# kerry-he/fsae-mpc

Measured on AMD Instinct MI355X. Metric: QP solves/sec (batched LTV-MPC, N=40 nx=5 nu=2 fp64), higher is better.
Workload: dtype f64

## Files before the change

### fsae-mpc_amd/csrc/qp_probe.h

```cpp
#pragma once
#include "qp_solve_kernel.h"

template <int T, int NB> __global__ __launch_bounds__(64) void syrk_probe_kernel(QpParams P, int reps) {
  const int b = blockIdx.x;
  extern __shared__ double lds[];
  Ctx k;
  ctx_setup<T>(k, P, b, lds);
  const QpSolveLds L = qp_solve_lds(T, NB, P.d.np);
  double* MB = lds + L.vecs;
  k.ring = MB + L.border + L.tiles; k.cof = k.ring + L.ring;
  for (int js = 0; js < k.JT; ++js) {
    const int ix = js * 64 + k.lane;
    rowp(k, R_D)[ix] = 1.0; rowp(k, R_W1)[ix] = 0.5; rowp(k, R_W2)[ix] = 0.25; rowp(k, R_W3)[ix] = 2.0;
  }
  __syncthreads();
  v4d acc[Tri<T>::NT];
  acc_init<T>(k, acc);
  const unsigned long long t0 = __builtin_amdgcn_s_memtime();
  for (int r = 0; r < reps; ++r) {
    Stream<T> st;
    st.open(k);
    pass_syrk<T, NB>(k, st, acc, vecp(k, V_P1), vecp(k, V_P2), vecp(k, V_P3), MB);
    st.close();
    __syncthreads();
// ... 60 lines not shown
  for (int r = 0; r < reps; ++r) {
    acc_init<T>(k, acc);
#pragma unroll
    for (int K = 0; K < T; ++K) {
#pragma unroll
      for (int p = 0; p < 4; ++p) if (k.q + 4 * p == k.c) acc[Tri<T>::idx(K, K)][p] += 20.0;
    }
    for (int i = k.lane; i < 16 * T; i += 64) RV[i] = 1.0 + (i & 15);
    __syncthreads();
    __builtin_amdgcn_sched_barrier(0);
    unsigned long long t0 = __builtin_amdgcn_s_memtime();
    reg_factor<T, 1>(k, acc, YL, 1e-30);
    __builtin_amdgcn_sched_barrier(0);
    unsigned long long t1 = __builtin_amdgcn_s_memtime();
    tt[0] += t1 - t0;
    v4d Yk, none = {0.0, 0.0, 0.0, 0.0};
#pragma unroll
    for (int K = 0; K < T; ++K) {
#pragma unroll
      for (int p = 0; p < 4; ++p) { Yk[p] = (k.q + 4 * p == k.c) ? 1.0 : 0.0; if (k.q + 4 * p == k.c) acc[Tri<T>::idx(K, K)][p] += 30.0; }
      diag_factor<DiagForm<T, 1>::form>(k, acc[Tri<T>::idx(K, K)], Yk, none, 1e-30);
      cs += Yk[0];
    }
    __builtin_amdgcn_sched_barrier(0);
    unsigned long long t2 = __builtin_amdgcn_s_memtime();
    tt[1] += t2 - t1;
#pragma unroll
    for (int K = 0; K < T; ++K) { tile_store(k, YL + K * 272, acc[Tri<T>::idx(K, K)]); __syncthreads(); acc[Tri<T>::idx(K, K)] = tile_load_t(k, YL + K * 272); }
    __builtin_amdgcn_sched_barrier(0);
    unsigned long long t3 = __builtin_amdgcn_s_memtime();
    tt[2] += t3 - t2;
    double y[T][4];
    vec_forward<T, true>(k, acc, YL, RV, y);
    WAVE_SYNC();
    vec_backward<T, true>(k, acc, YL, y, RV);
    WAVE_SYNC();
// ... 10 lines not shown
```

### fsae-mpc_amd/csrc/qp_rules.h

```cpp
#pragma once
#include <math.h>
#if defined(__HIPCC__)
#include <hip/hip_runtime.h>
#define QPR_HD __host__ __device__ __forceinline__
#else
#define QPR_HD inline
#endif
#ifndef QP_REFINE_ATTEMPTS
#define QP_REFINE_ATTEMPTS 3
#endif
template <int C> struct IC { static constexpr int value = C; };
#define QPR_GAMMA_F 0.99
#define QPR_STEP_BACKOFF 0.99999999
#define QPR_AMAX_UNSET 1e300
#define QPR_AMAX_SET 1e299
#define QPR_CORRECTOR_MIN_STEP 0.05
#define QPR_MU_FLOOR 1e-5
#define QPR_PROGRESS 0.9
#define QPR_STALL_SAVED 5
#define QPR_STALL_UNSAVED 25
#define QPR_DIVERGED_X 1e13
#define QPR_DIVERGED_Z 1e15
#define QPR_INFEASIBLE_RP 1e-6
#define QPR_RHO 1e6
// ... 18 lines not shown
  return o;
}
QPR_HD bool qpr_has_lower(bool valid, double l) { return valid && l > -INFINITY; }
QPR_HD bool qpr_has_upper(bool valid, double u) { return valid && u < INFINITY; }
QPR_HD double qpr_side_affine(double t, double z, double rp, double va, double& a_aff, double& s1, double& s2) {
  const double dt = va + rp, dz = -z - (z / t) * dt;
  if (dt < 0) a_aff = fmin(a_aff, -t / dt);  if (dz < 0) a_aff = fmin(a_aff, -z / dz);
  s1 += t * dz + z * dt; s2 += dt * dz;
  return dt * dz / t;
}
struct QprDir { double dt, dz; };
QPR_HD QprDir qpr_side_step(double t, double z, double rp, double va, double dv, double smu, double cw) {
  const double dta = va + rp, dza = -z - (z / t) * dta;
  const double c = smu - cw * dta * dza;
  QprDir o; o.dt = dv + rp; o.dz = -z + c / t - (z / t) * o.dt;
  return o;
}
struct QprBlock { double amax, bp, bdp, bd, bdd; };
QPR_HD QprBlock qpr_block_none() { QprBlock b; b.amax = QPR_AMAX_UNSET; b.bp = 0; b.bdp = 0; b.bd = 0; b.bdd = 0; return b; }
QPR_HD void qpr_side_block(double t, double z, const QprDir& d, QprBlock& b, double& q1, double& q2) {
  if (d.dt < 0 && -t / d.dt < b.amax) { b.amax = -t / d.dt; b.bp = t; b.bdp = d.dt; b.bd = z; b.bdd = d.dz; }
  if (d.dz < 0 && -z / d.dz < b.amax) { b.amax = -z / d.dz; b.bp = z; b.bdp = d.dz; b.bd = t; b.bdd = d.dt; }
  q1 += t * d.dz + z * d.dt; q2 += d.dt * d.dz;
}
struct QprCenter { double mu_aff, sigma, smu, cw; };
QPR_HD QprCenter qpr_centering(double gap, double cnt, double mu, double a_aff, double s1, double s2, double tol, double fval) {
  QprCenter o; o.mu_aff = fmax(0.0, gap + a_aff * (s1 + a_aff * s2)) / cnt;
  double sigma = mu > 0 ? (o.mu_aff / mu) * (o.mu_aff / mu) * (o.mu_aff / mu) : 0.0;
  if (sigma > 1.0) sigma = 1.0;
  const double mu_floor = QPR_MU_FLOOR * tol * fmax(1.0, fabs(fval)) / cnt;
// ... 97 lines not shown
```

### fsae-mpc_amd/csrc/qp_selftest.h

```cpp
#pragma once
#include <stdlib.h>
#include <stdio.h>
#include "qp_solve_kernel.h"

namespace {

__global__ void mfma_selftest_kernel(const double* Am, const double* Bm, double* Cm) {
  const int lane = threadIdx.x;
  const double a = Am[(lane & 15) * 4 + (lane >> 4)];
  const double bb = Bm[(lane >> 4) * 16 + (lane & 15)];
  v4d c = {0, 0, 0, 0};
  c = __builtin_amdgcn_mfma_f64_16x16x4f64(a, bb, c, 0, 0, 0);
#pragma unroll
  for (int p = 0; p < 4; ++p) Cm[((lane >> 4) + 4 * p) * 16 + (lane & 15)] = c[p];
}

DEVINL bool same_bits(double a, double b) { return __double_as_longlong(a) == __double_as_longlong(b) || (a != a && b != b); }
template <class OP> DEVINL double lds_grp16(double* sh, int lane, double v) {
  const int src[4] = {lane ^ 1, lane ^ 2, (lane & ~7) | (7 - (lane & 7)), (lane & ~15) | (15 - (lane & 15))};
#pragma unroll
  for (int s = 0; s < 4; ++s) {
    sh[lane] = v; __syncthreads();
    const double o = sh[src[s]]; __syncthreads();
    v = OP::f(v, o);
// ... 72 lines not shown
      double a[4] = {x[4], x[5], x[6], x[7]};
      wave_sum(a);
      int nb = 0;
#pragma unroll
      for (int i = 0; i < 4; ++i) nb += same_bits(a[i], wave_sum_zf(x[4 + i])) ? 0 : 1;
      if (nb && first < 0) first = 100 * 65;
      bad += nb;
    }
    if (bad != before && first_round < 0) first_round = r;
  }
  if (bad) {
    if (atomicAdd(&out[0], bad) == 0) { out[1] = first; out[2] = first_round; out[3] = lane; }
  }
}

template <int FORM> DEVINL int diag_factor_bad_vs_old(const Ctx& k, const v4d& U0, const v4d& R0, double floor_abs, const v4d& Uo, const v4d& Yo, const v4d& Ro, int bo) {
  v4d U = U0, R = R0, Y;
#pragma unroll
  for (int p = 0; p < 4; ++p) Y[p] = (k.q + 4 * p == k.c) ? 1.0 : 0.0;
  const int b = diag_factor<FORM>(k, U, Y, R, floor_abs);
  int bad = (b != bo) ? 1 : 0;
#pragma unroll
  for (int p = 0; p < 4; ++p)
    bad += (__double_as_longlong(U[p]) != __double_as_longlong(Uo[p])) + (__double_as_longlong(Y[p]) != __double_as_longlong(Yo[p])) +
           (__double_as_longlong(R[p]) != __double_as_longlong(Ro[p]));
  return bad;
}
__global__ __launch_bounds__(64) void diag_factor_selftest_kernel(const double* __restrict__ in, int ntiles, double floor_abs, int* __restrict__ out) {
  Ctx k = {};
  k.lane = threadIdx.x; k.c = k.lane & 15; k.q = k.lane >> 4;
  int bad = 0, first = -1, form = 0;
  for (int t = 0; t < ntiles; ++t) {
    v4d U0, R0, Uo, Ro, Yo;
#pragma unroll
    for (int p = 0; p < 4; ++p) {
      U0[p] = in[(size_t)t * 512 + (k.q + 4 * p) * 16 + k.c];
      R0[p] = in[(size_t)t * 512 + 256 + (k.q + 4 * p) * 16 + k.c];
      Yo[p] = (k.q + 4 * p == k.c) ? 1.0 : 0.0;
    }
    Uo = U0; Ro = R0;
    const int bo = diag_factor<0>(k, Uo, Yo, Ro, floor_abs);
    const int b1 = diag_factor_bad_vs_old<1>(k, U0, R0, floor_abs, Uo, Yo, Ro, bo);
    const int b2 = diag_factor_bad_vs_old<2>(k, U0, R0, floor_abs, Uo, Yo, Ro, bo);
    if ((b1 | b2) && first < 0) { first = t; form = b1 ? 1 : 2; }
    bad += b1 + b2;
  }
  if (bad) {
    if (atomicAdd(&out[0], bad) == 0) { out[1] = first; out[2] = form; out[3] = k.lane; }
  }
}

template <int T, int NB> __global__ __launch_bounds__(64) void initial_point_selftest_kernel(QpParams P, int* __restrict__ out) {
  extern __shared__ double lds[];
  Ctx k;
  (void)ctx_setup<T>(k, P, 0, lds);
  const QpSolveLds L = qp_solve_lds(T, NB, P.d.np);
  k.ring = lds + L.vecs + L.border + L.tiles;
  k.cof = k.ring + L.ring;
// ... 88 lines not shown
  (void)hipMemset(dout, 0, sizeof(hout));
  free(h);
  hipLaunchKernelGGL(lane_reduce_selftest_kernel, dim3(1), dim3(64), 0, 0, d, rounds, dout);
  hipError_t e = hipDeviceSynchronize();
  if (e == hipSuccess) e = hipMemcpy(hout, dout, sizeof(hout), hipMemcpyDeviceToHost);
  (void)hipFree(d); (void)hipFree(dout);
  if (e != hipSuccess) { snprintf(msg, msglen, "lane-reduce selftest: %s", hipGetErrorString(e)); return -1; }
  if (hout[0]) snprintf(msg, msglen, "lane reductions: %d mismatches, first: test %d (1/2/4/8: grp16 single / batched, 16: q, 64: wave, 65: wave_sum batch) op %d (sum/max/min) round %d lane %d",
                        hout[0], hout[1] / 100, hout[1] % 100, hout[2], hout[3]);
  return hout[0];
}

int qp_selftest_diag_factor(char* msg, int msglen) {
  const int ntiles = 64;
  const double floor_abs = 1e-9;
  double* h = (double*)malloc(sizeof(double) * ntiles * 512);
  if (!h) return -1;
  unsigned long long st = 0xD1B54A32D192ED03ull;
  auto rnd = [&]() { st = st * 6364136223846793005ull + 1442695040888963407ull; return ((unsigned)(st >> 33)) / 2147483648.0; };
  for (int t = 0; t < ntiles; ++t) {
    double* D = h + (size_t)t * 512; double* R = D + 256;
    double Q[16][16], sv[16];
    for (int i = 0; i < 16; ++i) for (int j = 0; j < 16; ++j) Q[i][j] = i == j ? 1.0 : 0.0;
    for (int r = 0; r < 3; ++r) {
      double v[16], vv = 0;
      for (int i = 0; i < 16; ++i) { v[i] = 2.0 * rnd() - 1.0; vv += v[i] * v[i]; }
      for (int i = 0; i < 16; ++i) {
        double qv = 0;
        for (int j = 0; j < 16; ++j) qv += Q[i][j] * v[j];
        for (int j = 0; j < 16; ++j) Q[i][j] -= 2.0 * qv * v[j] / vv;
      }
    }
    const double lc = 10.0 * (t < 61 ? t / 60.0 : 0.3);
    for (int i = 0; i < 16; ++i) sv[i] = pow(10.0, -lc * i / 15.0);
    for (int i = 0; i < 16; ++i) for (int j = 0; j < 16; ++j) {
      double a = 0;
      for (int l = 0; l < 16; ++l) a += Q[i][l] * sv[l] * Q[j][l];
      D[i * 16 + j] = a;
    }
    for (int i = 0; i < 16; ++i) for (int j = 0; j < i; ++j) D[i * 16 + j] = D[j * 16 + i];
    for (int i = 0; i < 256; ++i) R[i] = 20.0 * rnd() - 10.0;
    if (t == 61) for (int j = 0; j < 16; ++j) { D[6 * 16 + j] *= 1e-6; D[j * 16 + 6] *= 1e-6; }
    if (t == 62) { D[5 * 16 + 9] = NAN; D[9 * 16 + 5] = NAN; }
    if (t == 63) D[10 * 16 + 10] = INFINITY;
  }
  double* d = 0; int* dout = 0; int hout[4] = {0, 0, 0, 0};
  if (hipMalloc(&d, sizeof(double) * ntiles * 512) != hipSuccess || hipMalloc(&dout, sizeof(hout)) != hipSuccess) { free(h); if (d) (void)hipFree(d); return -1; }
  (void)hipMemcpy(d, h, sizeof(double) * ntiles * 512, hipMemcpyHostToDevice);
  (void)hipMemset(dout, 0, sizeof(hout));
  free(h);
  hipLaunchKernelGGL(diag_factor_selftest_kernel, dim3(1), dim3(64), 0, 0, d, ntiles, floor_abs, dout);
  hipError_t e = hipDeviceSynchronize();
  if (e == hipSuccess) e = hipMemcpy(hout, dout, sizeof(hout), hipMemcpyDeviceToHost);
  (void)hipFree(d); (void)hipFree(dout);
  if (e != hipSuccess) { snprintf(msg, msglen, "diag_factor selftest: %s", hipGetErrorString(e)); return -1; }
  if (hout[0]) snprintf(msg, msglen, "diag_factor forms: %d mismatches with the former form, first: tile %d form %d lane %d", hout[0], hout[1], hout[2], hout[3]);
  return hout[0];
}

template <int T, int NB> static hipError_t initial_point_launch(const QpParams& P, int* dout) {
  hipError_t e = hipFuncSetAttribute(reinterpret_cast<const void*>(&initial_point_selftest_kernel<T, NB>), hipFuncAttributeMaxDynamicSharedMemorySize, (int)P.d.lds_solve);
  if (e != hipSuccess) return e;
  hipLaunchKernelGGL((initial_point_selftest_kernel<T, NB>), dim3(1), dim3(64), P.d.lds_solve, 0, P, dout);
// ... 87 lines not shown
```

### fsae-mpc_amd/csrc/qp_solve_kernel.h

```cpp
#pragma once
#include "qp_solver.h"
#include "qp_lane.h"
#include "qp_rules.h"

#ifndef QP_SOLVE_PAIR
#define QP_SOLVE_PAIR 0
#endif
#ifndef QP_DIAG_FLAT
#define QP_DIAG_FLAT 1
#endif
#ifndef QP_SYRK_INTERLEAVE
#define QP_SYRK_INTERLEAVE 0
#endif
#ifndef QP_STARTUP_ATW
#define QP_STARTUP_ATW 0
#endif
#ifndef QP_SWEEP_BATCH
#define QP_SWEEP_BATCH 6
#endif

namespace {

template <int T> struct Tri {
  static constexpr int NT = T * (T + 1) / 2;
  __host__ __device__ static constexpr int idx(int I, int J) { return I * T - (I * (I - 1)) / 2 + (J - I); }
};

struct Ctx {
  int n, m, T, Kq, J, JB, JT, np, lane, c, q, nc, nb, ntr;
  const int* perm; const int* tcs; const int* aoff; const int* tend;
  const double* Aw; const double* Hw; const double* Ab; const double* Hb;
  double* rows;
  double* ring;
// ... 139 lines not shown
  DEVINL void load(const Ctx& k, const double* const* arr, int js) {
    const int jc = js < k.J ? js : k.J - 1;
#pragma unroll
    for (int a = 0; a < NA; ++a) reg[a] = arr[a][jc * 64 + k.lane];
  }
  DEVINL void commit(const Ctx& k) {
#pragma unroll
    for (int a = 0; a < NA; ++a) k.cof[a * 64 + k.lane] = reg[a];
  }
  DEVINL void read_pair(const Ctx& k, int s, v2d* out) const {
#pragma unroll
    for (int a = 0; a < NA; ++a) out[a] = *reinterpret_cast<const v2d*>(k.cof + a * 64 + k.q * 16 + (s & 15));
  }
};

template <int T, int NB> DEVINL void pass_syrk(const Ctx& k, Stream<T>& st, v4d* acc, double* P1, double* P2, double* P3, double* MB) {
  constexpr int NBB = NB > 0 ? NB : 1;
  constexpr int NA = 4 + NB;
  const int JS = k.J * 64;
  const double* arr[NA];
  arr[0] = rowp(k, R_D); arr[1] = rowp(k, R_W1); arr[2] = rowp(k, R_W2); arr[3] = rowp(k, R_W3);
#pragma unroll
  for (int e = 0; e < NB; ++e) arr[4 + e] = k.Ab + (size_t)e * JS;
  double p1[T], p2[T], p3[T];
  double pb[NBB][T], sbb[NBB][NBB], pwb[3][NBB];
#pragma unroll
  for (int t = 0; t < T; ++t) { p1[t] = 0; p2[t] = 0; p3[t] = 0; }
#pragma unroll
  for (int e = 0; e < NBB; ++e) {
#pragma unroll
    for (int t = 0; t < T; ++t) pb[e][t] = 0;
#pragma unroll
    for (int f = 0; f < NBB; ++f) sbb[e][f] = 0;
    pwb[0][e] = pwb[1][e] = pwb[2][e] = 0;
  }
  CoefStage<NA> cs;
  int tr = 0;
  st.start(k);
// ... 7 lines not shown
      for (int u = 0; u < 2; ++u) {
        v2d b[C], cf[NA];
        st.template next_pair<C>(k, b);
        cs.read_pair(k, 4 * tr + 2 * u, cf);
        asm volatile("" ::: "memory");
#if QP_SYRK_INTERLEAVE
        double a2[2][C];
#pragma unroll
        for (int h = 0; h < 2; ++h)
#pragma unroll
          for (int t = 0; t < C; ++t) a2[h][t] = cf[0][h] * b[t][h];
#endif
#pragma unroll
        for (int h = 0; h < 2; ++h) {
          double a[C], ab[NBB];
          const double dd = cf[0][h], w1 = cf[1][h], w2 = cf[2][h], w3 = cf[3][h];
#pragma unroll
          for (int e = 0; e < NB; ++e) ab[e] = cf[4 + e][h];
#pragma unroll
#if QP_SYRK_INTERLEAVE
          for (int t = 0; t < C; ++t) a[t] = a2[h][t];
#else
          for (int t = 0; t < C; ++t) a[t] = dd * b[t][h];
#endif
#pragma unroll
          for (int I = 0; I < C; ++I)
#pragma unroll
            for (int Jt = I; Jt < C; ++Jt)
              acc[Tri<T>::idx(I, Jt)] = __builtin_amdgcn_mfma_f64_16x16x4f64(a[I], b[Jt][h], acc[Tri<T>::idx(I, Jt)], 0, 0, 0);
#pragma unroll
          for (int t = 0; t < C; ++t) {
            p1[t] = fma(w1, b[t][h], p1[t]); p2[t] = fma(w2, b[t][h], p2[t]); p3[t] = fma(w3, b[t][h], p3[t]);
          }
#pragma unroll
          for (int e = 0; e < NB; ++e) {
            const double dab = dd * ab[e];
#pragma unroll
            for (int t = 0; t < C; ++t) pb[e][t] = fma(dab, b[t][h], pb[e][t]);
#pragma unroll
            for (int f = e; f < NB; ++f) sbb[e][f] = fma(dab, ab[f], sbb[e][f]);
            pwb[0][e] = fma(w1, ab[e], pwb[0][e]); pwb[1][e] = fma(w2, ab[e], pwb[1][e]); pwb[2][e] = fma(w3, ab[e], pwb[2][e]);
          }
#if QP_SYRK_INTERLEAVE
#pragma unroll
          for (int i = 0; i < C * (C + 1) / 2; ++i) {
            __builtin_amdgcn_sched_group_barrier(0x008, 1, 0);
            __builtin_amdgcn_sched_group_barrier(0x002, 2, 0);
          }
#endif
        }
      }
    }
  };
  if constexpr (T >= 1) phase(IC<1>{});
  if constexpr (T >= 2) phase(IC<2>{});
  if constexpr (T >= 3) phase(IC<3>{});
  if constexpr (T >= 4) phase(IC<4>{});
  if constexpr (T >= 5) phase(IC<5>{});
  if constexpr (T >= 6) phase(IC<6>{});
  if constexpr (T >= 7) phase(IC<7>{});
  if constexpr (T >= 8) phase(IC<8>{});
  if (k.ntr > 0) st.finish();
#pragma unroll
  for (int t = 0; t < T; ++t) {
    double v1 = q_sum(p1[t]), v2 = q_sum(p2[t]), v3 = q_sum(p3[t]);
    if (k.q == 0) { P1[16 * t + k.c] = v1; P2[16 * t + k.c] = v2; P3[16 * t + k.c] = v3; }
  }
#pragma unroll
  for (int e = 0; e < NB; ++e) {
#pragma unroll
    for (int t = 0; t < T; ++t) { const double vb = q_sum(pb[e][t]); if (k.q == 0) MB[e * k.np + 16 * t + k.c] = vb; }
    const double v1 = q_sum(pwb[0][e]), v2 = q_sum(pwb[1][e]), v3 = q_sum(pwb[2][e]);
    if (k.lane == 0) { P1[k.nc + e] = v1; P2[k.nc + e] = v2; P3[k.nc + e] = v3; }
#pragma unroll
    for (int f = 0; f < NB; ++f) {
      const double sv = q_sum(f >= e ? sbb[e][f] : sbb[f][e]);
      if (k.lane == 0) MB[e * k.np + k.nc + f] = sv;
    }
  }
}

template <int T, int NB, int NVEC, int FUSE> DEVINL void pass_Av(const Ctx& k, Stream<T>& st, const double* const* vin, double* const* rout, double* Pcor, double* Pcor2 = nullptr, const double* const* cfarr = nullptr) {
  constexpr int NBB = NB > 0 ? NB : 1;
  constexpr int NC = FUSE == 1 ? 6 : (FUSE >= 2 ? 3 : (FUSE == -1 ? 1 : 0));
  constexpr int NA = NC + NB;
  const int JS = k.J * 64;
  const double* arr[NA > 0 ? NA : 1];
  if (FUSE == 1) { arr[0] = rowp(k, R_RPL); arr[1] = rowp(k, R_CB1); arr[2] = rowp(k, R_CC1); arr[3] = rowp(k, R_RPU); arr[4] = rowp(k, R_CB2); arr[5] = rowp(k, R_CC2); }
// ... 165 lines not shown
  v4d Z;
#pragma unroll
  for (int p = 0; p < 4; ++p) Z[p] = slot[(k.q + 4 * p) * 17 + k.c];
  return Z;
}
DEVINL v4d tile_load_t(const Ctx& k, const double* slot) {
  v4d Z;
#pragma unroll
  for (int p = 0; p < 4; ++p) Z[p] = slot[k.c * 17 + k.q + 4 * p];
  return Z;
}

DEVINL double on_lanes(unsigned long long mask, double v, double otherwise) {
  return __builtin_amdgcn_inverse_ballot_w64(mask) ? v : otherwise;
}
template <int FORM> DEVINL int diag_factor(const Ctx& k, v4d& Ud, v4d& Yk, v4d& rk, double floor_abs) {
  constexpr bool FLAT = FORM >= 1;
  int bad = 0;
#pragma unroll
  for (int p = 0; p < 4; ++p) {
    const double d00 = rl(Ud[p], 4 * p + 0), d01 = rl(Ud[p], 4 * p + 1), d02 = rl(Ud[p], 4 * p + 2), d03 = rl(Ud[p], 4 * p + 3);
    const double d11 = rl(Ud[p], 16 + 4 * p + 1), d12 = rl(Ud[p], 16 + 4 * p + 2), d13 = rl(Ud[p], 16 + 4 * p + 3);
    const double d22 = rl(Ud[p], 32 + 4 * p + 2), d23 = rl(Ud[p], 32 + 4 * p + 3);
    const double d33 = rl(Ud[p], 48 + 4 * p + 3);
    auto piv = [&](double t) {
      if constexpr (FORM >= 2) {
        const bool low = !(t > floor_abs);
        bad |= (low & !(fabs(t) < INFINITY)) ? 1 : 0;
        t = low ? floor_abs : t;
      } else {
        if (!(t > floor_abs)) { if (!(fabs(t) < INFINITY)) bad = 1; t = floor_abs; }
// ... 14 lines not shown
    if constexpr (FLAT) {
      const unsigned long long L0 = 1ull << (4 * p), L1 = 1ull << (16 + 4 * p), L2 = 1ull << (32 + 4 * p), L3 = 1ull << (48 + 4 * p);
      double wa = on_lanes(L0, i0, 0.0);
      wa = on_lanes(L0 << 1, w10, wa); wa = on_lanes(L0 << 2, w20, wa); wa = on_lanes(L0 << 3, w30, wa);
      wa = on_lanes(L1 << 1, i1, wa); wa = on_lanes(L1 << 2, w21, wa); wa = on_lanes(L1 << 3, w31, wa);
      wa = on_lanes(L2 << 2, i2, wa); wa = on_lanes(L2 << 3, w32, wa);
      wa = on_lanes(L3 << 3, i3, wa);
      const v4d nu = __builtin_amdgcn_mfma_f64_16x16x4f64(wa, Ud[p], z, 0, 0, 0);
      Ud[p] = nu[p];
      double a = 0.0;
      if (p < 3) {
        a = on_lanes(0x0001000100010001ull * (0xFFFFull & (0xFFFFull << (4 * p + 4))), -Ud[p], 0.0);
        Ud = __builtin_amdgcn_mfma_f64_16x16x4f64(a, Ud[p], Ud, 0, 0, 0);
      }
      const v4d ny = __builtin_amdgcn_mfma_f64_16x16x4f64(wa, Yk[p], z, 0, 0, 0);
      const v4d nr = __builtin_amdgcn_mfma_f64_16x16x4f64(wa, rk[p], z, 0, 0, 0);
      Yk[p] = ny[p]; rk[p] = nr[p];
      if (p < 3) {
        Yk = __builtin_amdgcn_mfma_f64_16x16x4f64(a, Yk[p], Yk, 0, 0, 0);
        rk = __builtin_amdgcn_mfma_f64_16x16x4f64(a, rk[p], rk, 0, 0, 0);
      }
      if constexpr (FORM >= 2) asm("" : "+v"(bad));
    } else {
      const int a_ = k.c - 4 * p;
      double wa = 0.0;
      if (k.q == 0) wa = a_ == 0 ? i0 : (a_ == 1 ? w10 : (a_ == 2 ? w20 : (a_ == 3 ? w30 : 0.0)));
      if (k.q == 1) wa = a_ == 1 ? i1 : (a_ == 2 ? w21 : (a_ == 3 ? w31 : 0.0));
      if (k.q == 2) wa = a_ == 2 ? i2 : (a_ == 3 ? w32 : 0.0);
      if (k.q == 3) wa = a_ == 3 ? i3 : 0.0;
      const v4d nu = __builtin_amdgcn_mfma_f64_16x16x4f64(wa, Ud[p], z, 0, 0, 0);
      const v4d ny = __builtin_amdgcn_mfma_f64_16x16x4f64(wa, Yk[p], z, 0, 0, 0);
      const v4d nr = __builtin_amdgcn_mfma_f64_16x16x4f64(wa, rk[p], z, 0, 0, 0);
      Ud[p] = nu[p]; Yk[p] = ny[p]; rk[p] = nr[p];
      if (p < 3) {
        const double a = (k.c > 4 * p + 3) ? -Ud[p] : 0.0;
        Yk = __builtin_amdgcn_mfma_f64_16x16x4f64(a, Yk[p], Yk, 0, 0, 0);
        rk = __builtin_amdgcn_mfma_f64_16x16x4f64(a, rk[p], rk, 0, 0, 0);
        Ud = __builtin_amdgcn_mfma_f64_16x16x4f64(a, Ud[p], Ud, 0, 0, 0);
      }
    }
  }
#pragma unroll
  for (int p = 0; p < 4; ++p) if (k.c < k.q + 4 * p) Ud[p] = 0.0;
  return bad;
}

template <int T, int NB> struct DiagForm { static constexpr int form = (T == 5 && NB > 0) ? QP_DIAG_FLAT : 0; };

template <int T, int NB> struct SweepBatch { static constexpr int nsb = (T == 5 && NB > 0) ? QP_SWEEP_BATCH : 2; };

template <int T, int NB, int K> struct FactorStep {
  static DEVINL int run(const Ctx& k, v4d* acc, double* YL, double floor_abs) {
    v4d Yk, none = {0.0, 0.0, 0.0, 0.0};
#pragma unroll
    for (int p = 0; p < 4; ++p) Yk[p] = (k.q + 4 * p == k.c) ? 1.0 : 0.0;
    int bad = diag_factor<DiagForm<T, NB>::form>(k, acc[Tri<T>::idx(K, K)], Yk, none, floor_abs);
    tile_store(k, YL + K * 272, Yk);
    WAVE_SYNC();
    const v4d Wk = tile_load_t(k, YL + K * 272);
    const v4d& UKK = acc[Tri<T>::idx(K, K)];
#pragma unroll
    for (int Jt = K + 1; Jt < T; ++Jt) {
      v4d Rr = acc[Tri<T>::idx(K, Jt)];
      v4d Ukj = mfma4_new(Wk, Rr);
      mfma4_sub<T>(UKK, Ukj, Rr);
#pragma unroll
      for (int p = 0; p < 4; ++p) Ukj = __builtin_amdgcn_mfma_f64_16x16x4f64(Wk[p], Rr[p], Ukj, 0, 0, 0);
      acc[Tri<T>::idx(K, Jt)] = Ukj;
    }
#pragma unroll
    for (int I = K + 1; I < T; ++I) {
// ... 312 lines not shown
    WAVE_SYNC();
  }

  double saved_merit = INFINITY, best_res = INFINITY;
  int have_saved = 0, stall = 0;
  double* XS = ws + d.off_save;
  double* LAMS = ws + d.off_save + k.np;

  auto row1_body = [&](int ix, bool valid, double l, double u, double v, double tl, double tu, double zl, double zu,
                       double& s_gap, double& m_rp) {
    const QprRow o = qpr_row_weights(valid, l, u, v, tl, tu, zl, zu, s_gap, m_rp);
    aRPL[ix] = o.rpl; aRPU[ix] = o.rpu; rowp(k, R_CB1)[ix] = o.dl; rowp(k, R_CC1)[ix] = o.ccl;
    rowp(k, R_CB2)[ix] = o.du; rowp(k, R_CC2)[ix] = o.ccu;
    aD[ix] = o.D; aW1[ix] = o.W1; aW2[ix] = o.W2; aW3[ix] = o.W3;
  };
  struct Slot { int ix; bool valid; double l, u, v, tl, tu, zl, zu, va, vc, w2, rpl, rpu; };
  auto load_slot = [&](int js) {
    Slot s_;
    const int jc = js < JT ? js : JT - 1;
    s_.ix = jc * 64 + lane; s_.valid = js < JT && row_valid(k, jc);
    const int ix = s_.ix;
    s_.l = aL[ix]; s_.u = aU[ix]; s_.v = aV[ix]; s_.tl = aTL[ix]; s_.tu = aTU[ix]; s_.zl = aZL[ix]; s_.zu = aZU[ix];
    s_.va = aVA[ix]; s_.vc = aVC[ix]; s_.w2 = aW2[ix]; s_.rpl = aRPL[ix]; s_.rpu = aRPU[ix];
    return s_;
  };
  struct BoundVals { double va[2], vc[2], w2[2]; };
  auto bound_dirs = [&](BoundVals& bv) {
    for (int h = 0; h < 2; ++h) { const int i = lane + 64 * h; bv.va[h] = i < n ? R1[i] : 0.0; bv.vc[h] = i < n ? R2[i] : 0.0; }
  };
  constexpr int NSB = SweepBatch<T, NB>::nsb;
  auto sweep = [&](const BoundVals& bv, auto&& body) __attribute__((always_inline)) {
    for (int js0 = 0; js0 < JT; js0 += NSB) {
      Slot r[NSB];
#pragma unroll
      for (int e = 0; e < NSB; ++e) r[e] = load_slot(js0 + e);
#pragma unroll
      for (int e = 0; e < NSB; ++e) {
        const int js = js0 + e;
// ... 36 lines not shown
        const int i = lane + 64 * h;
        if (i < nc) {
          double r = R[i];
#pragma unroll
          for (int e = 0; e < NB; ++e) r = fma(-MB[e * k.np + i], xb[e], r);
          R[i] = r;
        }
      }
      if (lane == 0) {
#pragma unroll
        for (int e = 0; e < NB; ++e) R[nc + e] = xb[e];
      }
      WAVE_SYNC();
    }
  };
  auto factor_solve2 = [&](int it_now) __attribute__((always_inline)) -> int {
    double dmax_l = 0;
#pragma unroll
    for (int K = 0; K < T; ++K) {
      const int i = 16 * K + k.c;
      const int ix = (J + (i >> 6)) * 64 + (i & 63);
      const double dadd = i < n ? aD[ix] : 1.0;
      const bool mine = (k.q == (k.c & 3));
#pragma unroll
      for (int p = 0; p < 4; ++p)
        if (mine && p == (k.c >> 2)) { acc[Tri<T>::idx(K, K)][p] += dadd; dmax_l = fmax(dmax_l, acc[Tri<T>::idx(K, K)][p]); }
    }
    if (NB > 0) {
      for (int h = 0; h < 2; ++h) {
        const int i = lane + 64 * h;
        if (i < k.np) {
// ... 55 lines not shown
      for (int e = 0; e < NB; ++e) {
        double dd = S[e][e];
#pragma unroll
        for (int g2 = 0; g2 < e; ++g2) dd -= Ubb[g2][e] * Ubb[g2][e];
        if (!(dd > 1e-30 * dmax)) { if (!(fabs(dd) < INFINITY)) fbad = 1; dd = 1e-30 * dmax; }
        Ubb[e][e] = sqrt(dd);
#pragma unroll
        for (int f = e + 1; f < NB; ++f) {
          double tt = S[e][f];
#pragma unroll
          for (int g2 = 0; g2 < e; ++g2) tt -= Ubb[g2][e] * Ubb[g2][f];
          Ubb[e][f] = tt / Ubb[e][e];
        }
      }
    }
    if (fbad) return 1;
    {
      double y12[2][T][4];
      double (&y1)[T][4] = y12[0], (&y2)[T][4] = y12[1];
#if QP_SOLVE_PAIR
      { const double* const b12[2] = {R1, R2}; vec_forward<T, true, 2>(k, acc, YL, b12, y12); }
#else
      vec_forward<T, true>(k, acc, YL, R1, y1);
      vec_forward<T, true>(k, acc, YL, R2, y2);
#endif
      if (NB > 0) {
        WAVE_SYNC();
        vec_rows_store<T>(k, y1, R1); vec_rows_store<T>(k, y2, R2);
        WAVE_SYNC();
        border_solve(R1); border_solve(R2);
        vec_rows_load<T>(k, R1, y1); vec_rows_load<T>(k, R2, y2);
// ... 124 lines not shown
    }
    if (it >= P.max_iter) { flag = have_saved ? 2 : 1; break; }

    {
      const double* vin[2] = {R1, R2}; double* rout[2] = {aVA, aVC};
      pass_Av<T, NB, 2, 1>(k, st, vin, rout, P1);
    }
    BoundVals bv;
    bound_dirs(bv);
    bv.w2[0] = bv.w2[1] = 0.0;
    STAMP(7);
    double a_aff = 1.0, s1 = 0.0, s2 = 0.0;
    double wb[2] = {0.0, 0.0};
    auto row2_body = [&](const Slot& r, int js) {
      double w = 0.0;
      if (qpr_has_lower(r.valid, r.l)) w -= qpr_side_affine(r.tl, r.zl, r.rpl, r.va, a_aff, s1, s2);
      if (qpr_has_upper(r.valid, r.u)) w += qpr_side_affine(r.tu, r.zu, r.rpu, -r.va, a_aff, s1, s2);
      if (js == J) wb[0] = w;
      if (js == J + 1) wb[1] = w;
    };
    sweep(bv, row2_body);
    a_aff = wave_min(a_aff);
    s1 = wave_sum(s1); s2 = wave_sum(s2);
    const QprCenter cen = qpr_centering(gap, cnt, mu, a_aff, s1, s2, P.tol, fval); const double smu = cen.smu, cw = cen.cw;
    WAVE_SYNC();
    STAMP(8);
    if (cw != 0.0) {
    STAMP(9);
    for (int h = 0; h < 2; ++h) {
      const int i = lane + 64 * h;
      if (i < k.np) DX[i] = i < n ? P1[i] + wb[h] : 0.0;
    }
// ... 7 lines not shown
    }
    STAMP(11);
    } else {
      for (int i = lane; i < k.np; i += 64) DX[i] = 0.0;
      for (int js = 0; js < J; ++js) aW2[js * 64 + lane] = 0.0;
      WAVE_SYNC();
    }
    bound_dirs(bv);
    for (int h = 0; h < 2; ++h) { const int i = lane + 64 * h; bv.w2[h] = i < n ? DX[i] : 0.0; }
    for (int h = 0; h < 2; ++h) {
      const int i = lane + 64 * h;
      if (i < n) DX[i] = R1[i] + smu * R2[i] + DX[i];
    }
    QprBlock blk = qpr_block_none(); double q1 = 0.0, q2 = 0.0;
    double dvb[2] = {0.0, 0.0};
    auto row3a_body = [&](const Slot& r, int js) {
      const double dv = r.va + smu * r.vc + r.w2;
      if (js < J) aVC[r.ix] = dv;
      if (js == J) dvb[0] = dv;
      if (js == J + 1) dvb[1] = dv;
      if (qpr_has_lower(r.valid, r.l)) qpr_side_block(r.tl, r.zl, qpr_side_step(r.tl, r.zl, r.rpl, r.va, dv, smu, cw), blk, q1, q2);
      if (qpr_has_upper(r.valid, r.u)) qpr_side_block(r.tu, r.zu, qpr_side_step(r.tu, r.zu, r.rpu, -r.va, -dv, smu, cw), blk, q1, q2);
    };
    sweep(bv, row3a_body);
    const double amax_w = wave_min(blk.amax);
    double alpha = 1.0;
    if (amax_w < QPR_AMAX_SET) {
      const unsigned long long msk = __ballot(blk.amax == amax_w);
      const int src = __ffsll((long long)msk) - 1;
      q1 = wave_sum(q1); q2 = wave_sum(q2);
      alpha = qpr_step_length(gap, cnt, amax_w, q1, q2, rl(blk.bp, src), rl(blk.bdp, src), rl(blk.bd, src), rl(blk.bdd, src));
    }
#ifdef QP_DEBUG_DUMP
    if (P.dump && P.dump_stage == 5 && b == P.dump_iter && lane == 0 && it < 120) {
      double* o_ = P.dump + 16 * it;
      o_[8] = a_aff; o_[9] = cen.sigma; o_[10] = alpha; o_[11] = cw; o_[12] = amax_w; o_[13] = (double)stall;
    }
// ... 3 lines not shown
      c1 = wave_sum(c1); c2 = wave_sum(c2); c3 = wave_sum(c3); c4 = wave_sum(c4);
      if (lane == 0) {
        double* o_ = P.dump;
        o_[0] = a_aff; o_[1] = cen.mu_aff; o_[2] = cen.sigma; o_[3] = smu; o_[4] = cw; o_[5] = amax_w; o_[6] = alpha; o_[7] = gap; o_[8] = mu;
        o_[9] = c1; o_[10] = c2; o_[11] = c3; o_[12] = c4; o_[13] = s1; o_[14] = s2; o_[15] = q1; o_[16] = q2;
      }
      for (int i = lane; i < n; i += 64) { P.dump[32 + i] = DX[i]; P.dump[32 + n + i] = R1[i]; P.dump[32 + 2 * n + i] = R2[i]; P.dump[32 + 3 * n + i] = P1[i]; }
    }
#endif
    double xn = 0, zn = 0, s_gap = 0, m_rp = 0;
    auto row3b_body = [&](const Slot& r, int js) {
      if (js >= JT) return;
      const double dv = r.vc;
      double tl = r.tl, zl = r.zl, tu = r.tu, zu = r.zu;
      if (qpr_has_lower(r.valid, r.l)) {
        const QprDir s_ = qpr_side_step(tl, zl, r.rpl, r.va, dv, smu, cw);
        tl += alpha * s_.dt; zl += alpha * s_.dz;
        aTL[r.ix] = tl; aZL[r.ix] = zl;
        zn = fmax(zn, zl);
      }
      if (qpr_has_upper(r.valid, r.u)) {
        const QprDir s_ = qpr_side_step(tu, zu, r.rpu, -r.va, -dv, smu, cw);
        tu += alpha * s_.dt; zu += alpha * s_.dz;
        aTU[r.ix] = tu; aZU[r.ix] = zu;
        zn = fmax(zn, zu);
      }
      const double v = r.v + alpha * dv;
      aV[r.ix] = v;
      row1_body(r.ix, r.valid, r.l, r.u, v, tl, tu, zl, zu, s_gap, m_rp);
    };
    bv.vc[0] = dvb[0]; bv.vc[1] = dvb[1];
    sweep(bv, row3b_body);
    for (int h = 0; h < 2; ++h) {
      const int i = lane + 64 * h;
      if (i < n) { X[i] += alpha * DX[i]; xn = fmax(xn, fabs(X[i])); }
    }
    const double rp_prev = rp_rel;
    gap = wave_sum(s_gap);
    rp_rel = wave_max(m_rp);
    xn = wave_max(xn); zn = wave_max(zn);
    WAVE_SYNC();
    STAMP(12);
    if (qpr_exit_rule(xn, zn, rp_prev, fval, stall, have_saved, P.polish, flag)) break;
  }

  const bool v_current = flag == 0 || flag == 4;
// ... 28 lines not shown
      const int ix = js * 64 + lane;
      const double lam = aW3[ix]; const QprSide sd = qpr_working_side(row_valid(k, js), aL[ix], aU[ix], aV[ix], lam);
      PS[ix] = sd.side(); PY[ix] = (sd.active() && js < J) ? lam : 0.0;
    }
    for (int i = lane; i < k.np; i += 64) XS[i] = X[i];
    WAVE_SYNC();
    for (int attempt = 0; attempt < QP_REFINE_ATTEMPTS && flag_polished <= 0; ++attempt) {
    for (int js = 0; js < JT; ++js) {
      const int ix = js * 64 + lane;
      const double sd = PS[ix];
      PA[ix] = sd != 0.0 ? rho : 0.0; PB[ix] = qpr_target(sd, aL[ix], aU[ix]);
      aD[ix] = js < J ? PA[ix] : (sd != 0.0 ? pin : 0.0); aW1[ix] = 0.0; aW2[ix] = 0.0; PC[ix] = 0.0; PP[ix] = 0.0;
    }
    WAVE_SYNC();
    acc_init<T>(k, acc);
    pass_syrk<T, NB>(k, st, acc, P1, P2, P3, MB);
    WAVE_SYNC();
    for (int i = lane; i < k.np; i += 64) { R1[i] = 0.0; R2[i] = 0.0; }
    WAVE_SYNC();
    bool pok = factor_solve2(-1) == 0, retry = false;
    if (!pok) { flag_polished = -5; break; }
    for (int h = 0; h < 2; ++h) {
      const int i = lane + 64 * h;
      if (i < k.np) { const int ix = (J + (i >> 6)) * 64 + (i & 63); R2[i] = (i < n && PS[ix] != 0.0) ? PB[ix] : XS[i]; }
    }
    WAVE_SYNC();
    const double* cf_eval[3] = {PA, PB, PY};
    const double* cf_cg[3] = {PA, PZ0, PZ0};
    auto eval_zy = [&]() __attribute__((always_inline)) {
      const double* vin[1] = {R2}; double* rout[2] = {aVA, aVC};
      pass_Av<T, NB, 1, 3>(k, st, vin, rout, P1, P2, cf_eval);
      hx_full(R2);
      WAVE_SYNC();
    };
    if (pok) {
// ... 243 lines not shown
```

Baseline: 441,200.

## Drop unused diag-factor RHS, skip RHS work in refinement, reuse cached row ratios

```diff
diff --git a/fsae-mpc_amd/csrc/qp_probe.h b/fsae-mpc_amd/csrc/qp_probe.h
--- a/fsae-mpc_amd/csrc/qp_probe.h
+++ b/fsae-mpc_amd/csrc/qp_probe.h
@@ -98,12 +98,12 @@
     __builtin_amdgcn_sched_barrier(0);
     unsigned long long t1 = __builtin_amdgcn_s_memtime();
     tt[0] += t1 - t0;
-    v4d Yk, none = {0.0, 0.0, 0.0, 0.0};
+    v4d Yk;
 #pragma unroll
     for (int K = 0; K < T; ++K) {
 #pragma unroll
       for (int p = 0; p < 4; ++p) { Yk[p] = (k.q + 4 * p == k.c) ? 1.0 : 0.0; if (k.q + 4 * p == k.c) acc[Tri<T>::idx(K, K)][p] += 30.0; }
-      diag_factor<DiagForm<T, 1>::form>(k, acc[Tri<T>::idx(K, K)], Yk, none, 1e-30);
+      diag_factor<DiagForm<T, 1>::form>(k, acc[Tri<T>::idx(K, K)], Yk, 1e-30);
       cs += Yk[0];
     }
     __builtin_amdgcn_sched_barrier(0);
diff --git a/fsae-mpc_amd/csrc/qp_rules.h b/fsae-mpc_amd/csrc/qp_rules.h
--- a/fsae-mpc_amd/csrc/qp_rules.h
+++ b/fsae-mpc_amd/csrc/qp_rules.h
@@ -56,6 +56,18 @@
   const double dta = va + rp, dza = -z - (z / t) * dta;
   const double c = smu - cw * dta * dza;
   QprDir o; o.dt = dv + rp; o.dz = -z + c / t - (z / t) * o.dt;
+  return o;
+}
+QPR_HD double qpr_side_affine_d(double t, double z, double d, double rp, double va, double& a_aff, double& s1, double& s2) {
+  const double dt = va + rp, dz = -z - d * dt;
+  if (dt < 0) a_aff = fmin(a_aff, -t / dt);  if (dz < 0) a_aff = fmin(a_aff, -z / dz);
+  s1 += t * dz + z * dt; s2 += dt * dz;
+  return dt * dz / t;
+}
+QPR_HD QprDir qpr_side_step_d(double t, double z, double d, double rp, double va, double dv, double smu, double cw) {
+  const double dta = va + rp, dza = -z - d * dta;
+  const double c = smu - cw * dta * dza;
+  QprDir o; o.dt = dv + rp; o.dz = -z + c / t - d * o.dt;
   return o;
 }
 struct QprBlock { double amax, bp, bdp, bd, bdd; };
diff --git a/fsae-mpc_amd/csrc/qp_selftest.h b/fsae-mpc_amd/csrc/qp_selftest.h
--- a/fsae-mpc_amd/csrc/qp_selftest.h
+++ b/fsae-mpc_amd/csrc/qp_selftest.h
@@ -110,16 +110,15 @@
   }
 }
 
-template <int FORM> DEVINL int diag_factor_bad_vs_old(const Ctx& k, const v4d& U0, const v4d& R0, double floor_abs, const v4d& Uo, const v4d& Yo, const v4d& Ro, int bo) {
-  v4d U = U0, R = R0, Y;
+template <int FORM> DEVINL int diag_factor_bad_vs_old(const Ctx& k, const v4d& U0, double floor_abs, const v4d& Uo, const v4d& Yo, int bo) {
+  v4d U = U0, Y;
 #pragma unroll
   for (int p = 0; p < 4; ++p) Y[p] = (k.q + 4 * p == k.c) ? 1.0 : 0.0;
-  const int b = diag_factor<FORM>(k, U, Y, R, floor_abs);
+  const int b = diag_factor<FORM>(k, U, Y, floor_abs);
   int bad = (b != bo) ? 1 : 0;
 #pragma unroll
   for (int p = 0; p < 4; ++p)
-    bad += (__double_as_longlong(U[p]) != __double_as_longlong(Uo[p])) + (__double_as_longlong(Y[p]) != __double_as_longlong(Yo[p])) +
-           (__double_as_longlong(R[p]) != __double_as_longlong(Ro[p]));
+    bad += (__double_as_longlong(U[p]) != __double_as_longlong(Uo[p])) + (__double_as_longlong(Y[p]) != __double_as_longlong(Yo[p]));
   return bad;
 }
 __global__ __launch_bounds__(64) void diag_factor_selftest_kernel(const double* __restrict__ in, int ntiles, double floor_abs, int* __restrict__ out) {
@@ -127,17 +126,16 @@
   k.lane = threadIdx.x; k.c = k.lane & 15; k.q = k.lane >> 4;
   int bad = 0, first = -1, form = 0;
   for (int t = 0; t < ntiles; ++t) {
-    v4d U0, R0, Uo, Ro, Yo;
+    v4d U0, Uo, Yo;
 #pragma unroll
     for (int p = 0; p < 4; ++p) {
-      U0[p] = in[(size_t)t * 512 + (k.q + 4 * p) * 16 + k.c];
-      R0[p] = in[(size_t)t * 512 + 256 + (k.q + 4 * p) * 16 + k.c];
+      U0[p] = in[(size_t)t * 256 + (k.q + 4 * p) * 16 + k.c];
       Yo[p] = (k.q + 4 * p == k.c) ? 1.0 : 0.0;
     }
-    Uo = U0; Ro = R0;
-    const int bo = diag_factor<0>(k, Uo, Yo, Ro, floor_abs);
-    const int b1 = diag_factor_bad_vs_old<1>(k, U0, R0, floor_abs, Uo, Yo, Ro, bo);
-    const int b2 = diag_factor_bad_vs_old<2>(k, U0, R0, floor_abs, Uo, Yo, Ro, bo);
+    Uo = U0;
+    const int bo = diag_factor<0>(k, Uo, Yo, floor_abs);
+    const int b1 = diag_factor_bad_vs_old<1>(k, U0, floor_abs, Uo, Yo, bo);
+    const int b2 = diag_factor_bad_vs_old<2>(k, U0, floor_abs, Uo, Yo, bo);
     if ((b1 | b2) && first < 0) { first = t; form = b1 ? 1 : 2; }
     bad += b1 + b2;
   }
@@ -256,12 +254,12 @@
 int qp_selftest_diag_factor(char* msg, int msglen) {
   const int ntiles = 64;
   const double floor_abs = 1e-9;
-  double* h = (double*)malloc(sizeof(double) * ntiles * 512);
+  double* h = (double*)malloc(sizeof(double) * ntiles * 256);
   if (!h) return -1;
   unsigned long long st = 0xD1B54A32D192ED03ull;
   auto rnd = [&]() { st = st * 6364136223846793005ull + 1442695040888963407ull; return ((unsigned)(st >> 33)) / 2147483648.0; };
   for (int t = 0; t < ntiles; ++t) {
-    double* D = h + (size_t)t * 512; double* R = D + 256;
+    double* D = h + (size_t)t * 256;
     double Q[16][16], sv[16];
     for (int i = 0; i < 16; ++i) for (int j = 0; j < 16; ++j) Q[i][j] = i == j ? 1.0 : 0.0;
     for (int r = 0; r < 3; ++r) {
@@ -281,14 +279,13 @@
       D[i * 16 + j] = a;
     }
     for (int i = 0; i < 16; ++i) for (int j = 0; j < i; ++j) D[i * 16 + j] = D[j * 16 + i];
-    for (int i = 0; i < 256; ++i) R[i] = 20.0 * rnd() - 10.0;
     if (t == 61) for (int j = 0; j < 16; ++j) { D[6 * 16 + j] *= 1e-6; D[j * 16 + 6] *= 1e-6; }
     if (t == 62) { D[5 * 16 + 9] = NAN; D[9 * 16 + 5] = NAN; }
     if (t == 63) D[10 * 16 + 10] = INFINITY;
   }
   double* d = 0; int* dout = 0; int hout[4] = {0, 0, 0, 0};
-  if (hipMalloc(&d, sizeof(double) * ntiles * 512) != hipSuccess || hipMalloc(&dout, sizeof(hout)) != hipSuccess) { free(h); if (d) (void)hipFree(d); return -1; }
-  (void)hipMemcpy(d, h, sizeof(double) * ntiles * 512, hipMemcpyHostToDevice);
+  if (hipMalloc(&d, sizeof(double) * ntiles * 256) != hipSuccess || hipMalloc(&dout, sizeof(hout)) != hipSuccess) { free(h); if (d) (void)hipFree(d); return -1; }
+  (void)hipMemcpy(d, h, sizeof(double) * ntiles * 256, hipMemcpyHostToDevice);
   (void)hipMemset(dout, 0, sizeof(hout));
   free(h);
   hipLaunchKernelGGL(diag_factor_selftest_kernel, dim3(1), dim3(64), 0, 0, d, ntiles, floor_abs, dout);
diff --git a/fsae-mpc_amd/csrc/qp_solve_kernel.h b/fsae-mpc_amd/csrc/qp_solve_kernel.h
--- a/fsae-mpc_amd/csrc/qp_solve_kernel.h
+++ b/fsae-mpc_amd/csrc/qp_solve_kernel.h
@@ -17,6 +17,9 @@
 #endif
 #ifndef QP_SWEEP_BATCH
 #define QP_SWEEP_BATCH 6
+#endif
+#ifndef QP_REFINE_FACTOR_ONLY
+#define QP_REFINE_FACTOR_ONLY 1
 #endif
 
 namespace {
@@ -186,14 +189,16 @@
   }
 };
 
-template <int T, int NB> DEVINL void pass_syrk(const Ctx& k, Stream<T>& st, v4d* acc, double* P1, double* P2, double* P3, double* MB) {
+template <int T, int NB, bool RHS = true> DEVINL void pass_syrk(const Ctx& k, Stream<T>& st, v4d* acc, double* P1, double* P2, double* P3, double* MB) {
   constexpr int NBB = NB > 0 ? NB : 1;
-  constexpr int NA = 4 + NB;
+  constexpr int NW = RHS ? 4 : 1;
+  constexpr int NA = NW + NB;
   const int JS = k.J * 64;
   const double* arr[NA];
-  arr[0] = rowp(k, R_D); arr[1] = rowp(k, R_W1); arr[2] = rowp(k, R_W2); arr[3] = rowp(k, R_W3);
-#pragma unroll
-  for (int e = 0; e < NB; ++e) arr[4 + e] = k.Ab + (size_t)e * JS;
+  arr[0] = rowp(k, R_D);
+  if constexpr (RHS) { arr[1] = rowp(k, R_W1); arr[2] = rowp(k, R_W2); arr[3] = rowp(k, R_W3); }
+#pragma unroll
+  for (int e = 0; e < NB; ++e) arr[NW + e] = k.Ab + (size_t)e * JS;
   double p1[T], p2[T], p3[T];
   double pb[NBB][T], sbb[NBB][NBB], pwb[3][NBB];
 #pragma unroll
@@ -231,9 +236,9 @@
 #pragma unroll
         for (int h = 0; h < 2; ++h) {
           double a[C], ab[NBB];
-          const double dd = cf[0][h], w1 = cf[1][h], w2 = cf[2][h], w3 = cf[3][h];
-#pragma unroll
-          for (int e = 0; e < NB; ++e) ab[e] = cf[4 + e][h];
+          const double dd = cf[0][h], w1 = RHS ? cf[NW > 1 ? 1 : 0][h] : 0.0, w2 = RHS ? cf[NW > 2 ? 2 : 0][h] : 0.0, w3 = RHS ? cf[NW > 3 ? 3 : 0][h] : 0.0;
+#pragma unroll
+          for (int e = 0; e < NB; ++e) ab[e] = cf[NW + e][h];
 #pragma unroll
 #if QP_SYRK_INTERLEAVE
           for (int t = 0; t < C; ++t) a[t] = a2[h][t];
@@ -245,9 +250,11 @@
 #pragma unroll
             for (int Jt = I; Jt < C; ++Jt)
               acc[Tri<T>::idx(I, Jt)] = __builtin_amdgcn_mfma_f64_16x16x4f64(a[I], b[Jt][h], acc[Tri<T>::idx(I, Jt)], 0, 0, 0);
-#pragma unroll
-          for (int t = 0; t < C; ++t) {
-            p1[t] = fma(w1, b[t][h], p1[t]); p2[t] = fma(w2, b[t][h], p2[t]); p3[t] = fma(w3, b[t][h], p3[t]);
+          if constexpr (RHS) {
+#pragma unroll
+            for (int t = 0; t < C; ++t) {
+              p1[t] = fma(w1, b[t][h], p1[t]); p2[t] = fma(w2, b[t][h], p2[t]); p3[t] = fma(w3, b[t][h], p3[t]);
+            }
           }
 #pragma unroll
           for (int e = 0; e < NB; ++e) {
@@ -256,7 +263,7 @@
             for (int t = 0; t < C; ++t) pb[e][t] = fma(dab, b[t][h], pb[e][t]);
 #pragma unroll
             for (int f = e; f < NB; ++f) sbb[e][f] = fma(dab, ab[f], sbb[e][f]);
-            pwb[0][e] = fma(w1, ab[e], pwb[0][e]); pwb[1][e] = fma(w2, ab[e], pwb[1][e]); pwb[2][e] = fma(w3, ab[e], pwb[2][e]);
+            if constexpr (RHS) { pwb[0][e] = fma(w1, ab[e], pwb[0][e]); pwb[1][e] = fma(w2, ab[e], pwb[1][e]); pwb[2][e] = fma(w3, ab[e], pwb[2][e]); }
           }
 #if QP_SYRK_INTERLEAVE
 #pragma unroll
@@ -278,17 +285,21 @@
   if constexpr (T >= 7) phase(IC<7>{});
   if constexpr (T >= 8) phase(IC<8>{});
   if (k.ntr > 0) st.finish();
-#pragma unroll
-  for (int t = 0; t < T; ++t) {
-    double v1 = q_sum(p1[t]), v2 = q_sum(p2[t]), v3 = q_sum(p3[t]);
-    if (k.q == 0) { P1[16 * t + k.c] = v1; P2[16 * t + k.c] = v2; P3[16 * t + k.c] = v3; }
+  if constexpr (RHS) {
+#pragma unroll
+    for (int t = 0; t < T; ++t) {
+      double v1 = q_sum(p1[t]), v2 = q_sum(p2[t]), v3 = q_sum(p3[t]);
+      if (k.q == 0) { P1[16 * t + k.c] = v1; P2[16 * t + k.c] = v2; P3[16 * t + k.c] = v3; }
+    }
   }
 #pragma unroll
   for (int e = 0; e < NB; ++e) {
 #pragma unroll
     for (int t = 0; t < T; ++t) { const double vb = q_sum(pb[e][t]); if (k.q == 0) MB[e * k.np + 16 * t + k.c] = vb; }
-    const double v1 = q_sum(pwb[0][e]), v2 = q_sum(pwb[1][e]), v3 = q_sum(pwb[2][e]);
-    if (k.lane == 0) { P1[k.nc + e] = v1; P2[k.nc + e] = v2; P3[k.nc + e] = v3; }
+    if constexpr (RHS) {
+      const double v1 = q_sum(pwb[0][e]), v2 = q_sum(pwb[1][e]), v3 = q_sum(pwb[2][e]);
+      if (k.lane == 0) { P1[k.nc + e] = v1; P2[k.nc + e] = v2; P3[k.nc + e] = v3; }
+    }
 #pragma unroll
     for (int f = 0; f < NB; ++f) {
       const double sv = q_sum(f >= e ? sbb[e][f] : sbb[f][e]);
@@ -484,7 +495,7 @@
 DEVINL double on_lanes(unsigned long long mask, double v, double otherwise) {
   return __builtin_amdgcn_inverse_ballot_w64(mask) ? v : otherwise;
 }
-template <int FORM> DEVINL int diag_factor(const Ctx& k, v4d& Ud, v4d& Yk, v4d& rk, double floor_abs) {
+template <int FORM> DEVINL int diag_factor(const Ctx& k, v4d& Ud, v4d& Yk, double floor_abs) {
   constexpr bool FLAT = FORM >= 1;
   int bad = 0;
 #pragma unroll
@@ -529,12 +540,8 @@
         Ud = __builtin_amdgcn_mfma_f64_16x16x4f64(a, Ud[p], Ud, 0, 0, 0);
       }
       const v4d ny = __builtin_amdgcn_mfma_f64_16x16x4f64(wa, Yk[p], z, 0, 0, 0);
-      const v4d nr = __builtin_amdgcn_mfma_f64_16x16x4f64(wa, rk[p], z, 0, 0, 0);
-      Yk[p] = ny[p]; rk[p] = nr[p];
-      if (p < 3) {
-        Yk = __builtin_amdgcn_mfma_f64_16x16x4f64(a, Yk[p], Yk, 0, 0, 0);
-        rk = __builtin_amdgcn_mfma_f64_16x16x4f64(a, rk[p], rk, 0, 0, 0);
-      }
+      Yk[p] = ny[p];
+      if (p < 3) Yk = __builtin_amdgcn_mfma_f64_16x16x4f64(a, Yk[p], Yk, 0, 0, 0);
       if constexpr (FORM >= 2) asm("" : "+v"(bad));
     } else {
       const int a_ = k.c - 4 * p;
@@ -545,12 +552,10 @@
       if (k.q == 3) wa = a_ == 3 ? i3 : 0.0;
       const v4d nu = __builtin_amdgcn_mfma_f64_16x16x4f64(wa, Ud[p], z, 0, 0, 0);
       const v4d ny = __builtin_amdgcn_mfma_f64_16x16x4f64(wa, Yk[p], z, 0, 0, 0);
-      const v4d nr = __builtin_amdgcn_mfma_f64_16x16x4f64(wa, rk[p], z, 0, 0, 0);
-      Ud[p] = nu[p]; Yk[p] = ny[p]; rk[p] = nr[p];
+      Ud[p] = nu[p]; Yk[p] = ny[p];
       if (p < 3) {
         const double a = (k.c > 4 * p + 3) ? -Ud[p] : 0.0;
         Yk = __builtin_amdgcn_mfma_f64_16x16x4f64(a, Yk[p], Yk, 0, 0, 0);
-        rk = __builtin_amdgcn_mfma_f64_16x16x4f64(a, rk[p], rk, 0, 0, 0);
         Ud = __builtin_amdgcn_mfma_f64_16x16x4f64(a, Ud[p], Ud, 0, 0, 0);
       }
     }
@@ -564,12 +569,20 @@
 
 template <int T, int NB> struct SweepBatch { static constexpr int nsb = (T == 5 && NB > 0) ? QP_SWEEP_BATCH : 2; };
 
+#ifndef QP_ROW_REUSE
+#define QP_ROW_REUSE 1
+#endif
+template <int T, int NB> struct RowReuse { static constexpr bool on = QP_ROW_REUSE && T == 5; };
+#ifndef QP_ROW_HANDOVER
+#define QP_ROW_HANDOVER 1
+#endif
+
 template <int T, int NB, int K> struct FactorStep {
   static DEVINL int run(const Ctx& k, v4d* acc, double* YL, double floor_abs) {
-    v4d Yk, none = {0.0, 0.0, 0.0, 0.0};
+    v4d Yk;
 #pragma unroll
     for (int p = 0; p < 4; ++p) Yk[p] = (k.q + 4 * p == k.c) ? 1.0 : 0.0;
-    int bad = diag_factor<DiagForm<T, NB>::form>(k, acc[Tri<T>::idx(K, K)], Yk, none, floor_abs);
+    int bad = diag_factor<DiagForm<T, NB>::form>(k, acc[Tri<T>::idx(K, K)], Yk, floor_abs);
     tile_store(k, YL + K * 272, Yk);
     WAVE_SYNC();
     const v4d Wk = tile_load_t(k, YL + K * 272);
@@ -912,7 +925,8 @@
     rowp(k, R_CB2)[ix] = o.du; rowp(k, R_CC2)[ix] = o.ccu;
     aD[ix] = o.D; aW1[ix] = o.W1; aW2[ix] = o.W2; aW3[ix] = o.W3;
   };
-  struct Slot { int ix; bool valid; double l, u, v, tl, tu, zl, zu, va, vc, w2, rpl, rpu; };
+  constexpr bool REUSE = RowReuse<T, NB>::on, HANDOVER = REUSE && QP_ROW_HANDOVER;
+  struct Slot { int ix; bool valid; double l, u, v, tl, tu, zl, zu, va, vc, w2, rpl, rpu, dl, du; };
   auto load_slot = [&](int js) {
     Slot s_;
     const int jc = js < JT ? js : JT - 1;
@@ -920,6 +934,7 @@
     const int ix = s_.ix;
     s_.l = aL[ix]; s_.u = aU[ix]; s_.v = aV[ix]; s_.tl = aTL[ix]; s_.tu = aTU[ix]; s_.zl = aZL[ix]; s_.zu = aZU[ix];
     s_.va = aVA[ix]; s_.vc = aVC[ix]; s_.w2 = aW2[ix]; s_.rpl = aRPL[ix]; s_.rpu = aRPU[ix];
+    if constexpr (REUSE) { s_.dl = rowp(k, R_CB1)[ix]; s_.du = rowp(k, R_CB2)[ix]; } else { s_.dl = 0.0; s_.du = 0.0; }
     return s_;
   };
   struct BoundVals { double va[2], vc[2], w2[2]; };
@@ -986,7 +1001,7 @@
       WAVE_SYNC();
     }
   };
-  auto factor_solve2 = [&](int it_now) __attribute__((always_inline)) -> int {
+  auto factor_M = [&](int it_now) __attribute__((always_inline)) -> int {
     double dmax_l = 0;
 #pragma unroll
     for (int K = 0; K < T; ++K) {
@@ -1072,7 +1087,10 @@
         }
       }
     }
-    if (fbad) return 1;
+    return fbad ? 1 : 0;
+  };
+  auto factor_solve2 = [&](int it_now) __attribute__((always_inline)) -> int {
+    if (factor_M(it_now)) return 1;
     {
       double y12[2][T][4];
       double (&y1)[T][4] = y12[0], (&y2)[T][4] = y12[1];
@@ -1227,8 +1245,13 @@
     double wb[2] = {0.0, 0.0};
     auto row2_body = [&](const Slot& r, int js) {
       double w = 0.0;
-      if (qpr_has_lower(r.valid, r.l)) w -= qpr_side_affine(r.tl, r.zl, r.rpl, r.va, a_aff, s1, s2);
-      if (qpr_has_upper(r.valid, r.u)) w += qpr_side_affine(r.tu, r.zu, r.rpu, -r.va, a_aff, s1, s2);
+      if constexpr (REUSE) {
+        if (qpr_has_lower(r.valid, r.l)) w -= qpr_side_affine_d(r.tl, r.zl, r.dl, r.rpl, r.va, a_aff, s1, s2);
+        if (qpr_has_upper(r.valid, r.u)) w += qpr_side_affine_d(r.tu, r.zu, r.du, r.rpu, -r.va, a_aff, s1, s2);
+      } else {
+        if (qpr_has_lower(r.valid, r.l)) w -= qpr_side_affine(r.tl, r.zl, r.rpl, r.va, a_aff, s1, s2);
+        if (qpr_has_upper(r.valid, r.u)) w += qpr_side_affine(r.tu, r.zu, r.rpu, -r.va, a_aff, s1, s2);
+      }
       if (js == J) wb[0] = w;
       if (js == J + 1) wb[1] = w;
     };
@@ -1266,13 +1289,25 @@
     }
     QprBlock blk = qpr_block_none(); double q1 = 0.0, q2 = 0.0;
     double dvb[2] = {0.0, 0.0};
+    double dzb[2][2] = {{0.0, 0.0}, {0.0, 0.0}};
     auto row3a_body = [&](const Slot& r, int js) {
       const double dv = r.va + smu * r.vc + r.w2;
       if (js < J) aVC[r.ix] = dv;
       if (js == J) dvb[0] = dv;
       if (js == J + 1) dvb[1] = dv;
-      if (qpr_has_lower(r.valid, r.l)) qpr_side_block(r.tl, r.zl, qpr_side_step(r.tl, r.zl, r.rpl, r.va, dv, smu, cw), blk, q1, q2);
-      if (qpr_has_upper(r.valid, r.u)) qpr_side_block(r.tu, r.zu, qpr_side_step(r.tu, r.zu, r.rpu, -r.va, -dv, smu, cw), blk, q1, q2);
+      if constexpr (REUSE) {
+        double dzl = 0.0, dzu = 0.0;
+        if (qpr_has_lower(r.valid, r.l)) { const QprDir s_ = qpr_side_step_d(r.tl, r.zl, r.dl, r.rpl, r.va, dv, smu, cw); dzl = s_.dz; qpr_side_block(r.tl, r.zl, s_, blk, q1, q2); }
+        if (qpr_has_upper(r.valid, r.u)) { const QprDir s_ = qpr_side_step_d(r.tu, r.zu, r.du, r.rpu, -r.va, -dv, smu, cw); dzu = s_.dz; qpr_side_block(r.tu, r.zu, s_, blk, q1, q2); }
+        if constexpr (HANDOVER) {
+          if (js < J) { aVA[r.ix] = dzl; aW2[r.ix] = dzu; }
+#pragma unroll
+          for (int h = 0; h < 2; ++h) if (js == J + h) { dzb[h][0] = dzl; dzb[h][1] = dzu; }
+        }
+      } else {
+        if (qpr_has_lower(r.valid, r.l)) qpr_side_block(r.tl, r.zl, qpr_side_step(r.tl, r.zl, r.rpl, r.va, dv, smu, cw), blk, q1, q2);
+        if (qpr_has_upper(r.valid, r.u)) qpr_side_block(r.tu, r.zu, qpr_side_step(r.tu, r.zu, r.rpu, -r.va, -dv, smu, cw), blk, q1, q2);
+      }
     };
     sweep(bv, row3a_body);
     const double amax_w = wave_min(blk.amax);
@@ -1306,13 +1341,19 @@
       const double dv = r.vc;
       double tl = r.tl, zl = r.zl, tu = r.tu, zu = r.zu;
       if (qpr_has_lower(r.valid, r.l)) {
-        const QprDir s_ = qpr_side_step(tl, zl, r.rpl, r.va, dv, smu, cw);
+        QprDir s_;
+        if constexpr (HANDOVER) { s_.dt = dv + r.rpl; s_.dz = r.va; }
+        else if constexpr (REUSE) s_ = qpr_side_step_d(tl, zl, r.dl, r.rpl, r.va, dv, smu, cw);
+        else s_ = qpr_side_step(tl, zl, r.rpl, r.va, dv, smu, cw);
         tl += alpha * s_.dt; zl += alpha * s_.dz;
         aTL[r.ix] = tl; aZL[r.ix] = zl;
         zn = fmax(zn, zl);
       }
       if (qpr_has_upper(r.valid, r.u)) {
-        const QprDir s_ = qpr_side_step(tu, zu, r.rpu, -r.va, -dv, smu, cw);
+        QprDir s_;
+        if constexpr (HANDOVER) { s_.dt = -dv + r.rpu; s_.dz = r.w2; }
+        else if constexpr (REUSE) s_ = qpr_side_step_d(tu, zu, r.du, r.rpu, -r.va, -dv, smu, cw);
+        else s_ = qpr_side_step(tu, zu, r.rpu, -r.va, -dv, smu, cw);
         tu += alpha * s_.dt; zu += alpha * s_.dz;
         aTU[r.ix] = tu; aZU[r.ix] = zu;
         zn = fmax(zn, zu);
@@ -1322,6 +1363,10 @@
       row1_body(r.ix, r.valid, r.l, r.u, v, tl, tu, zl, zu, s_gap, m_rp);
     };
     bv.vc[0] = dvb[0]; bv.vc[1] = dvb[1];
+    if constexpr (HANDOVER) {
+#pragma unroll
+      for (int h = 0; h < 2; ++h) { bv.va[h] = dzb[h][0]; bv.w2[h] = dzb[h][1]; }
+    }
     sweep(bv, row3b_body);
     for (int h = 0; h < 2; ++h) {
       const int i = lane + 64 * h;
@@ -1380,11 +1425,17 @@
     }
     WAVE_SYNC();
     acc_init<T>(k, acc);
+#if QP_REFINE_FACTOR_ONLY
+    pass_syrk<T, NB, false>(k, st, acc, P1, P2, P3, MB);
+    WAVE_SYNC();
+    bool pok = factor_M(-1) == 0, retry = false;
+#else
     pass_syrk<T, NB>(k, st, acc, P1, P2, P3, MB);
     WAVE_SYNC();
     for (int i = lane; i < k.np; i += 64) { R1[i] = 0.0; R2[i] = 0.0; }
     WAVE_SYNC();
     bool pok = factor_solve2(-1) == 0, retry = false;
+#endif
     if (!pok) { flag_polished = -5; break; }
     for (int h = 0; h < 2; ++h) {
       const int i = lane + 64 * h;
```

New measurement: 445,100 (median of 4 runs). Within noise of the previous version (+0.9%).
